# NVIDIA-Merlin/NVTabular

Hardware: AMD Instinct MI355X
Metric: rows/sec + GB/s (Criteo Categorify+FillMissing+Normalize fit+transform, HBM-resident) (higher is better)
Workload: dtype int32 keys -> int64 labels; fp64 moments/normalize; 1 GPU; synthetic Criteo-day0: 26 int32 categorical (Criteo-1TB cardinalities, Zipf) + 13 int32 continuous, nulls as Arrow bitmaps; Categorify + FillMissing + Normalize, fit + transform; rows_per_gpu=45000000, algorithmic_bytes_per_row=624, tie_break=value (count desc, value asc), artifacts=deferred (no parquet I/O inside the timed region)

## Files before the change

### nvtabular_amd/csrc/nvt_range_count.hip

```cpp
#include <cstdio>
#include <cstdlib>
#include <type_traits>

#include "nvt_common.hpp"
#include "nvt_internal.hpp"
#include "nvt_prof.hpp"
#include "nvt_range.hpp"

namespace nvt {

namespace {

constexpr int32_t kEmpty = INT32_MIN;
constexpr int kRpBS = 1024;
constexpr int kRpG = NVT_RANGE_WGS;
constexpr int kRpBinWords = 20480;
constexpr int kRpLine = 16;
constexpr int kRpMaxNbLog2 = 10;
constexpr int kHotSlotsR = NVT_HOT_IMAGE_WORDS;
constexpr int kHotBucketsR = kHotSlotsR / 2;
constexpr int kRpProbe = 512;
#ifndef NVT_RP_MAX_EPOCH
#define NVT_RP_MAX_EPOCH 8
#endif
constexpr unsigned kRpMaxEpoch = NVT_RP_MAX_EPOCH;
#ifndef NVT_RANGE_U
#define NVT_RANGE_U 2
#endif
constexpr unsigned long long kStAgg = 1ull << 62, kStPrefix = 2ull << 62,
                             kStMask = (1ull << 62) - 1ull;

__device__ __forceinline__ uint32_t hot_bucket_r(int32_t key) { return hot_image_bucket(key, kHotBucketsR - 1); }

template <bool PW>
__device__ __forceinline__ uint32_t rp_fine(const RangeMap &map, int32_t key) {
  if constexpr (PW) return map.fine(key);
  else return map.template fine_staged<false>(key);
}


template <int U, int NBL, bool PW>
__global__ __launch_bounds__(kRpBS) void rp_partition_kernel(
    const int32_t *__restrict__ keys, const uint8_t *__restrict__ valid, uint64_t n,
    const int32_t *__restrict__ aux, int nb_log2_rt, uint32_t region_cap, int32_t *__restrict__ regions,
    uint32_t *__restrict__ fills, unsigned *__restrict__ hot_cnt, uint64_t *state,
    unsigned long long *__restrict__ clr_status, unsigned *__restrict__ clr_hist) {
  const int nb_log2 = NBL ? NBL : nb_log2_rt;
  {
    const unsigned nst = (1u << nb_log2) + 8u;
    for (unsigned i = blockIdx.x * kRpBS + threadIdx.x; i < nst; i += kRpG * kRpBS) clr_status[i] = 0ull;
    if (blockIdx.x == kRpG - 1 && threadIdx.x < 256) clr_hist[threadIdx.x] = 0u;
  }
  __shared__ int4 hot[kHotBucketsR];
  __shared__ int32_t bins[kRpBinWords];
  __shared__ unsigned fill[1 << kRpMaxNbLog2], flushed[1 << kRpMaxNbLog2];
  __shared__ unsigned scratch[kWave];
  __shared__ unsigned long long s_nulls, s_sent;
  __shared__ unsigned s_ovf;
  const unsigned NB = 1u << nb_log2, CAP = (unsigned)kRpBinWords >> nb_log2;
  const unsigned g = blockIdx.x, lane = lane_id();
  int32_t fill0 = 0x5A5A5A5A, fill1 = fill0 + 1;
  while (hot_bucket_r(fill1) == hot_bucket_r(fill0)) ++fill1;
  const uint32_t fb0 = hot_bucket_r(fill0);
  for (int i = threadIdx.x; i < kHotBucketsR; i += kRpBS) {
    const int2 k2 = reinterpret_cast<const int2 *>(aux)[i];
    const int32_t fk = (uint32_t)i != fb0 ? fill0 : fill1;
    hot[i] = make_int4(k2.x == kEmpty ? fk : k2.x, k2.y == kEmpty ? fk : k2.y, 0, 0);
  }
  for (unsigned i = threadIdx.x; i < NB; i += kRpBS) {
    fill[i] = 0;
    flushed[i] = 0;
  }
  if (threadIdx.x == 0) {
    s_nulls = 0;
    s_sent = 0;
    s_ovf = 0;
  }
  RangeMap map = load_map(aux);
  __shared__ uint32_t s_pieces[kRpPwWords];
  stage_pieces(map, s_pieces, threadIdx.x, kRpBS);
  __syncthreads();

  const unsigned BPW = NB / (kRpBS / kWave);
  __shared__ unsigned s_epoch[2];
  if (threadIdx.x < 2) s_epoch[threadIdx.x] = 0;
  auto flush_bins = [&](bool all, unsigned parity) {
    {
      const bool owner = lane < BPW;
      const unsigned wave_base = (threadIdx.x / kWave) * BPW;
      const unsigned t = wave_base + (owner ? lane : 0u);
      const unsigned fr = owner ? fill[t] : 0u;
      const unsigned done0 = owner ? flushed[t] : 0u;
      const bool over = fr > CAP;
      const unsigned f = over ? CAP : fr;
      const unsigned nfl = (all || over) ? f : (f / kRpLine) * kRpLine;
      const unsigned padn = over ? ((0u - (done0 + fr)) & (kRpLine - 1u)) : 0u;
      {
        const unsigned long long ob = __ballot(over);
        const unsigned long long hb = __ballot(fr * 2u > CAP);
        if (lane == 0 && (ob | hb))
          atomicAdd(&s_epoch[parity], ((unsigned)__popcll(ob) << 8) | (hb ? 1u : 0u));
      }
      unsigned long long todo = __ballot(nfl > 0);
      const unsigned sub = lane >> 4, l16 = lane & 15;
      while (todo) {
        int sel = -1;
#pragma unroll
        for (unsigned q = 0; q < 4; ++q) {
          const int bit = todo ? (int)__ffsll((long long)todo) - 1 : -1;
          if (todo) todo &= todo - 1;
          sel = (q == sub) ? bit : sel;
        }
        const unsigned src = sel >= 0 ? (unsigned)sel : 0u;
        const unsigned fb = __shfl(f, src, 64), nb_out = __shfl(nfl, src, 64);
        const unsigned done = __shfl(done0, src, 64), frb = __shfl(fr, src, 64), pb = __shfl(padn, src, 64);
        if (sel >= 0) {
          const unsigned bin = wave_base + (unsigned)sel;
          const int32_t *bsrc = bins + bin * CAP;
          const unsigned reach = frb > fb ? done + frb + pb : done + nb_out;
          if (reach > region_cap) {
            if (l16 == 0) atomicOr(&s_ovf, 1u);
          } else {
            int32_t *dst = regions + ((uint64_t)bin * kRpG + g) * region_cap + done;
            for (unsigned u = l16; u < nb_out; u += kRpLine) dst[u] = bsrc[u];
            if (l16 < pb) dst[frb + l16] = kEmpty;
          }
          const unsigned rem = fb - nb_out;
          int32_t keep = 0;
          if (l16 < rem) keep = bsrc[nb_out + l16];
          if (l16 < rem) bins[bin * CAP + l16] = keep;
        }
      }
      if (owner) {
        fill[t] = f - nfl;
        flushed[t] = over ? done0 + fr + padn : done0 + nfl;
      }
    }
  };

  const uint64_t nvec = (n + 3) / 4, nfull = n / 4;
  const uint64_t per = (nvec + kRpG - 1) / kRpG;
  const uint64_t v_lo = (uint64_t)g * per;
  const uint64_t v_hi = v_lo + per < nvec ? v_lo + per : nvec;
  const uint64_t vf_hi = v_hi < nfull ? v_hi : nfull;
  unsigned long long nulls = 0, notvalid = 0;
  unsigned long long empties = 0;
  const uint8_t *vsrc = valid != nullptr ? valid : reinterpret_cast<const uint8_t *>(keys);
  const unsigned vor = valid != nullptr ? 0u : 0xFFu;
  const uint64_t v_last = vf_hi > v_lo ? vf_hi - 1 : 0;
  int4 npack[U];
  unsigned nbyte[U];
  auto issue = [&](uint64_t v0) {
#pragma unroll
    for (int u = 0; u < U; ++u) {
      uint64_t v = v0 + (uint64_t)u * kRpBS;
      v = v < v_last ? v : v_last;
      npack[u] = reinterpret_cast<const int4 *>(keys)[v];
      nbyte[u] = (unsigned)vsrc[v >> 1];
    }
  };
  bool tail_round = false;
  int4 tpack = make_int4(0, 0, 0, 0);
  unsigned tok = 0, tin = 0;
  if (nfull < nvec && nfull >= v_lo && nfull < v_hi) {
    tail_round = true;
    if (threadIdx.x == 0) {
      int32_t kk[4] = {0, 0, 0, 0};
      for (int j = 0; j < 4; ++j) {
        const uint64_t i = nfull * 4 + j;
        if (i < n) {
          tin |= 1u << j;
          if (bit_valid(valid, i)) {
            kk[j] = keys[i];
            tok |= 1u << j;
          }
        }
      }
      tpack = make_int4(kk[0], kk[1], kk[2], kk[3]);
    }
  }
  unsigned R = 1, since = 0, epoch = 0;
  if (vf_hi > v_lo) issue(v_lo + threadIdx.x);
  for (uint64_t v0 = v_lo; v0 < vf_hi || tail_round; v0 += (uint64_t)kRpBS * U) {
    const bool is_tail = !(v0 < vf_hi);
    int32_t kv[4 * U];
    unsigned oks[U], ins[U];
#pragma unroll
    for (int u = 0; u < U; ++u) {
      const uint64_t v = v0 + (uint64_t)u * kRpBS + threadIdx.x;
      const bool present = !is_tail && v < vf_hi;
      kv[4 * u + 0] = npack[u].x;
      kv[4 * u + 1] = npack[u].y;
      kv[4 * u + 2] = npack[u].z;
      kv[4 * u + 3] = npack[u].w;
      oks[u] = present ? (((nbyte[u] | vor) >> (((unsigned)v & 1u) * 4u)) & 0xFu) : 0u;
      ins[u] = present ? 0xFu : 0u;
    }
    if (is_tail) {
      tail_round = false;
      kv[0] = tpack.x;
      kv[1] = tpack.y;
      kv[2] = tpack.z;
      kv[3] = tpack.w;
      oks[0] = tok;
      ins[0] = tin;
    } else {
      issue(v0 + (uint64_t)kRpBS * U + threadIdx.x);
    }
    unsigned pend = 0;
#pragma unroll
    for (int u = 0; u < U; ++u) {
      const unsigned ok = oks[u], in = ins[u];
      nulls += __popc(in & ~ok);
      notvalid += 4u - __popc(ok);
      int32_t kp[4];
      int4 hb[4];
      uint32_t sa[4];
#pragma unroll
      for (int j = 0; j < 4; ++j) {
        const int32_t m = (int32_t)(ok << (31 - j)) >> 31;
        kp[j] = (kv[4 * u + j] & m) | (kEmpty & ~m);
        sa[j] = hot_bucket_r(kp[j]);
      }
#pragma unroll
      for (int j = 0; j < 4; ++j) {
        const int2 kk2 = *reinterpret_cast<const int2 *>(&hot[sa[j]]);
        hb[j].x = kk2.x;
        hb[j].y = kk2.y;
      }
#pragma unroll
      for (int j = 0; j < 4; ++j) {
        const int q = 4 * u + j;
        const int32_t key = kp[j];
        const bool hx = hb[j].x == key, hy = hb[j].y == key;
        const bool hit = hx | hy;
        const bool is_e = key == kEmpty;
        empties += (unsigned)__popcll(__ballot(is_e));
        unsigned *cnt = reinterpret_cast<unsigned *>(&hot[sa[j]]) + (hy ? 3 : 2);
        atomicAdd(hit ? cnt : &scratch[lane], hit ? 1u : 0u);
        pend |= ((!hit & !is_e) ? 1u : 0u) << q;
      }
    }
    if (s_ovf) pend = 0;
#pragma unroll
    for (int q = 0; q < 4 * U; ++q) {
      if ((pend >> q) & 1) {
        const unsigned bkt = rp_fine<PW>(map, kv[q]) >> 14;
        const unsigned pos = atomicAdd(&fill[bkt], 1u);
        if (pos < CAP) {
          bins[bkt * CAP + pos] = kv[q];
        } else {
          const unsigned at = flushed[bkt] + pos;
          if (at < region_cap)
            regions[((uint64_t)bkt * kRpG + g) * region_cap + at] = kv[q];
          else
            atomicOr(&s_ovf, 1u);
        }
      }
    }
    if (++since >= R) {
      __syncthreads();
      flush_bins(false, epoch & 1u);
      if (threadIdx.x == 0) s_epoch[(epoch + 1u) & 1u] = 0;
      __syncthreads();
      const unsigned fl = s_epoch[epoch & 1u];
#ifndef NVT_RP_GROW_DIV
#define NVT_RP_GROW_DIV 16u
#endif
#ifndef NVT_RP_SHRINK_DIV
#define NVT_RP_SHRINK_DIV 4u
#endif
      if ((fl >> 8) > NB / NVT_RP_SHRINK_DIV) R = R > 1u ? R / 2u : 1u;
      else if ((fl >> 8) <= NB / NVT_RP_GROW_DIV) R = R < kRpMaxEpoch ? R * 2u : R;
      ++epoch;
      since = 0;
    }
  }
  __syncthreads();
  flush_bins(true, epoch & 1u);
  __syncthreads();
  for (unsigned b = threadIdx.x; b < NB; b += kRpBS) fills[(uint64_t)b * kRpG + g] = flushed[b];
  for (int i = threadIdx.x; i < kHotBucketsR; i += kRpBS) {
    const int4 hbk = hot[i];
    reinterpret_cast<uint2 *>(hot_cnt + (uint64_t)g * kHotSlotsR)[i] = make_uint2((unsigned)hbk.z, (unsigned)hbk.w);
  }
#pragma unroll
  for (int off = 32; off > 0; off >>= 1) {
    nulls += __shfl_down(nulls, off, 64);
    notvalid += __shfl_down(notvalid, off, 64);
  }
  if (lane == 0) {
    if (nulls) atomicAdd(&s_nulls, nulls);
    const unsigned long long sent = empties - notvalid;
    if (sent) atomicAdd(&s_sent, sent);
  }
  __syncthreads();
  if (threadIdx.x == 0) {
    if (s_nulls) atomicAdd((unsigned long long *)&state[NVT_ST_NULLS], s_nulls);
    if (s_sent) atomicAdd((unsigned long long *)&state[NVT_ST_SENTINEL], s_sent);
    if (s_ovf) atomicOr((unsigned long long *)&state[NVT_ST_OVERFLOW], 1ull | NVT_OVF_REGION);
    if (g == 0) atomicAdd((unsigned long long *)&state[NVT_ST_ROWS], (unsigned long long)n);
  }
}

constexpr int kTotGroups = 16;
__global__ __launch_bounds__(64 * kTotGroups) void hot_totals_kernel(
    const unsigned *__restrict__ hot_cnt, int nblocks, unsigned *__restrict__ hot_tot) {
  __shared__ unsigned part[kTotGroups][64];
  const unsigned l = threadIdx.x & 63, g = threadIdx.x >> 6;
  const unsigned slot = blockIdx.x * 64 + l;
  unsigned t = 0;
#pragma unroll 16
  for (int b = (int)g; b < nblocks; b += kTotGroups) t += hot_cnt[(uint64_t)b * kHotSlotsR + slot];
  part[g][l] = t;
  __syncthreads();
  if (g != 0) return;
  unsigned tot = 0;
#pragma unroll
  for (int q = 0; q < kTotGroups; ++q) tot += part[q][l];
  hot_tot[slot] = tot;
}

template <bool PW>
__global__ __launch_bounds__(kRpBS) void rp_count_kernel(
    const int32_t *__restrict__ regions, const uint32_t *__restrict__ fills, uint32_t region_cap,
    const int32_t *__restrict__ aux, const unsigned *__restrict__ hot_tot, int nb_log2,
    unsigned long long *status, unsigned *ticket, int32_t *__restrict__ out_keys,
    int64_t *__restrict__ out_cnt, uint64_t out_cap, unsigned *cls_hist,
    unsigned long long *__restrict__ range_table, uint32_t *__restrict__ out_slots, uint64_t *state) {
  constexpr int NSL = kRpSlots + kRpTail;
  constexpr int NW = kRpBS / kWave;
  __shared__ int32_t lkeys[NSL];
  __shared__ unsigned lcnt[NSL];
  __shared__ unsigned run_len[kRpG];
  __shared__ unsigned hist[256];
  __shared__ unsigned wtot[NW];
  __shared__ unsigned lovf, s_b, s_bad, s_mx;
  __shared__ unsigned long long s_base;
  if (threadIdx.x == 0) {
    s_b = atomicAdd(ticket, 1u);
    lovf = 0;
    s_mx = 0;
  }
  for (int i = threadIdx.x; i < NSL; i += kRpBS) {
    lkeys[i] = kEmpty;
    lcnt[i] = 0;
  }
  if (threadIdx.x < 256) hist[threadIdx.x] = 0;
  __syncthreads();
  const unsigned b = s_b, NB = 1u << nb_log2;
  const unsigned lane = lane_id(), w = threadIdx.x / kWave;
  RangeMap map = load_map(aux);
  __shared__ uint32_t s_pieces[kRpPwWords];
  stage_pieces(map, s_pieces, threadIdx.x, kRpBS);
  const bool skip = (state[NVT_ST_OVERFLOW] & 1ull) != 0;
  if (threadIdx.x < kRpG) {
    const unsigned len = fills[(uint64_t)b * kRpG + threadIdx.x];
    run_len[threadIdx.x] = (skip || len > region_cap) ? 0u : len;
  }
  __syncthreads();
  bool failed = skip;
  auto insert_from = [&](int32_t key, unsigned wgt, uint32_t s) {
#pragma unroll 4
    for (int p = 0; p < kRpProbe; ++p, ++s) {
      if (s >= (uint32_t)NSL) break;
      int32_t cur = lkeys[s];
      if (cur == kEmpty) {
        cur = atomicCAS(&lkeys[s], kEmpty, key);
        if (cur == kEmpty) cur = key;
      }
      if (cur == key) {
        atomicAdd(&lcnt[s], wgt);
        return;
      }
    }
    failed = true;
  };
  const unsigned hot_h0 = (unsigned)aux[NVT_RANGE_AUX_HOTSTART + b], hot_h1 = (unsigned)aux[NVT_RANGE_AUX_HOTSTART + b + 1];
  int32_t hot_key0 = kEmpty;
  unsigned hot_tot0 = 0;
  if (hot_h0 + threadIdx.x < hot_h1) {
    const unsigned slot = reinterpret_cast<const unsigned short *>(aux + NVT_RANGE_AUX_HOTORDER)[hot_h0 + threadIdx.x];
    hot_key0 = aux[slot];
    hot_tot0 = hot_tot[slot];
  }
  {
    __shared__ unsigned s_pre[kRpG + 2];
    __shared__ unsigned s_wsum[kRpG / kWave];
    static_assert(kRpG % kWave == 0 && kRpG <= kRpBS, "one thread per run");
    {
      unsigned len = 0, inc = 0;
      if (threadIdx.x < kRpG) {
        len = run_len[threadIdx.x];
        inc = len;
#pragma unroll
        for (int off = 1; off < 64; off <<= 1) {
          const unsigned o = __shfl_up(inc, off, 64);
          if (lane >= (unsigned)off) inc += o;
        }
        if (lane == 63) s_wsum[w] = inc;
      }
      __syncthreads();
      if (threadIdx.x < kRpG) {
        unsigned wb = 0;
        for (unsigned q = 0; q < w; ++q) wb += s_wsum[q];
        s_pre[threadIdx.x] = wb + inc - len;
        if (threadIdx.x == kRpG - 1) s_pre[kRpG] = wb + inc;
      }
    }
    __syncthreads();
    const unsigned *pre = s_pre;
    const unsigned all_keys = pre[kRpG];
    const unsigned share = (all_keys + NW - 1) / NW;
    const unsigned f_lo = w * share < all_keys ? w * share : all_keys;
    const unsigned total = f_lo + share < all_keys ? f_lo + share : all_keys;
    const int32_t *rbase = regions + (uint64_t)b * kRpG * region_cap;
#ifndef NVT_RP_GB
#define NVT_RP_GB 8
#endif
    constexpr int GB = NVT_RP_GB;
    unsigned r = 0;
    {
      const unsigned f = f_lo + lane < all_keys ? f_lo + lane : (all_keys ? all_keys - 1 : 0);
      unsigned lo = 0, hi = kRpG;
      while (hi - lo > 1) {
        const unsigned mid = (lo + hi) >> 1;
        if (pre[mid] <= f) lo = mid; else hi = mid;
      }
      r = lo;
    }
    unsigned r_lo = pre[r], r_hi = pre[r + 1];
    for (unsigned f0 = f_lo; f0 < total && !failed; f0 += GB * kWave) {
      int32_t kk[GB];
#pragma unroll
      for (int u = 0; u < GB; ++u) {
        const unsigned f = f0 + u * kWave + lane;
        kk[u] = kEmpty;
        if (f < total) {
          while (f >= r_hi) {
            ++r;
            r_lo = r_hi;
            r_hi = pre[r + 1];
          }
          kk[u] = rbase[(uint64_t)r * region_cap + (f - r_lo)];
        }
      }
      uint32_t hs[GB];
      int32_t cur[GB];
#pragma unroll
      for (int u = 0; u < GB; ++u) hs[u] = rp_fine<PW>(map, kk[u]) & (kRpSlots - 1);
#pragma unroll
      for (int u = 0; u < GB; ++u) cur[u] = lkeys[hs[u]];
#pragma unroll
      for (int u = 0; u < GB; ++u) {
        if (cur[u] == kEmpty && kk[u] != kEmpty) {
          cur[u] = atomicCAS(&lkeys[hs[u]], kEmpty, kk[u]);
          cur[u] = cur[u] == kEmpty ? kk[u] : cur[u];
        }
      }
      unsigned todo = 0;
#pragma unroll
      for (int u = 0; u < GB; ++u) {
        if (kk[u] == kEmpty) continue;
        if (cur[u] == kk[u])
          atomicAdd(&lcnt[hs[u]], 1u);
        else
          todo |= 1u << u;
      }
      int32_t wkey = 0;
      uint32_t ws = 0;
      int wp = 0;
      bool walking = false;
      while (true) {
        if (!walking && todo) {
          const int u = (int)__ffs((int)todo) - 1;
          wkey = kk[0];
          ws = hs[0];
#pragma unroll
          for (int q = 1; q < GB; ++q) {
            wkey = u == q ? kk[q] : wkey;
            ws = u == q ? hs[q] : ws;
          }
          todo &= todo - 1u;
          ++ws;
          wp = 1;
          walking = true;
        }
        if (!__any(walking)) break;
        if (walking) {
          if (ws >= (uint32_t)NSL || wp >= kRpProbe) {
            failed = true;
            walking = false;
          } else {
            int32_t c = lkeys[ws];
            if (c == kEmpty) {
              c = atomicCAS(&lkeys[ws], kEmpty, wkey);
              if (c == kEmpty) c = wkey;
            }
            if (c == wkey) {
              atomicAdd(&lcnt[ws], 1u);
              walking = false;
            } else {
              ++ws;
              ++wp;
            }
          }
        }
      }
    }
  }
  {
    if (hot_key0 != kEmpty && hot_tot0 > 0 && !failed)
      insert_from(hot_key0, hot_tot0, rp_fine<PW>(map, hot_key0) & (kRpSlots - 1));
    const unsigned short *order = reinterpret_cast<const unsigned short *>(aux + NVT_RANGE_AUX_HOTORDER);
    for (unsigned jx = hot_h0 + threadIdx.x + kRpBS; jx < hot_h1; jx += kRpBS) {
      const unsigned slot = order[jx];
      const int32_t key = aux[slot];
      const unsigned tot = hot_tot[slot];
      if (key != kEmpty && tot > 0 && !failed) insert_from(key, tot, rp_fine<PW>(map, key) & (kRpSlots - 1));
    }
  }
  if (failed) atomicOr(&lovf, 1u);
  __syncthreads();
  if (threadIdx.x == 0)
    s_bad = (lovf != 0 ||
             (__hip_atomic_load(&state[NVT_ST_OVERFLOW], __ATOMIC_RELAXED,
                                __HIP_MEMORY_SCOPE_AGENT) & 1ull))
                ? 1u : 0u;
  __syncthreads();
  const bool bad = s_bad != 0;
  const unsigned long long sent_rows = b == 0 ? state[NVT_ST_SENTINEL] : 0ull;
  const unsigned extra = sent_rows > 0 ? 1u : 0u;
  constexpr int ITER = (NSL + kRpBS - 1) / kRpBS;
  unsigned mine = 0;
  for (int it = 0; it < ITER; ++it) {
    const int i = it * kRpBS + (int)threadIdx.x;
    const bool occ = i < NSL && lkeys[i] != kEmpty;
    mine += (unsigned)__popcll(__ballot(occ));
  }
  if (lane == 0) wtot[w] = mine;
  __syncthreads();
  unsigned E = extra;
  for (int q = 0; q < NW; ++q) E += wtot[q];
  const bool full = E > (unsigned)(kRpSlots / 4 * 3);
  if (bad || full) E = 0;
  if (w == 0) {
    unsigned long long excl = 0;
    if (lane == 0)
      __hip_atomic_store(&status[b], (b == 0 ? kStPrefix : kStAgg) | (unsigned long long)E,
                         __ATOMIC_RELAXED, __HIP_MEMORY_SCOPE_AGENT);
    if (b > 0) {
      int top = (int)b - 1;
      while (true) {
        const int idx = top - (int)lane;
        unsigned long long v = kStPrefix;
        if (idx >= 0) {
          do {
            v = __hip_atomic_load(&status[idx], __ATOMIC_RELAXED, __HIP_MEMORY_SCOPE_AGENT);
#ifndef NVT_RP_SLEEP
#define NVT_RP_SLEEP 1
#endif
            if ((v >> 62) == 0) __builtin_amdgcn_s_sleep(NVT_RP_SLEEP);
          } while ((v >> 62) == 0);
        }
        const unsigned long long isp = __ballot((v >> 62) == 2);
        const int first = isp ? (int)__ffsll((long long)isp) - 1 : 64;
        unsigned long long add = ((int)lane <= first) ? (v & kStMask) : 0ull;
#pragma unroll
        for (int off = 32; off > 0; off >>= 1) add += __shfl_down(add, off, 64);
        excl += __shfl(add, 0, 64);
        if (isp) break;
        top -= 64;
      }
      if (lane == 0)
        __hip_atomic_store(&status[b], kStPrefix | (excl + E), __ATOMIC_RELAXED,
                           __HIP_MEMORY_SCOPE_AGENT);
    }
    if (lane == 0) s_base = excl;
  }
  __syncthreads();
  const unsigned long long base = s_base;
  if (b == NB - 1 && threadIdx.x == 0) {
    if (base + E > out_cap) {
      atomicOr((unsigned long long *)&state[NVT_ST_OVERFLOW], 2ull);
      state[NVT_ST_NEED] = base + E;
    } else {
      state[NVT_ST_OCCUPIED] = base + E;
    }
  }
  if (bad || full) {
    if (threadIdx.x == 0 && (lovf != 0 || full))
      atomicOr((unsigned long long *)&state[NVT_ST_OVERFLOW],
               1ull | (lovf != 0 ? NVT_OVF_PROBE : 0ull) | (full ? NVT_OVF_FULL : 0ull));
    return;
  }
  if (base + E > out_cap) return;
  if (extra && threadIdx.x == 0) {
    out_keys[base] = kEmpty;
    out_cnt[base] = (int64_t)sent_rows;
    if (out_slots != nullptr) out_slots[base] = 0xFFFFFFFFu;
    const unsigned cls = sent_rows < 255 ? (unsigned)sent_rows : 255u;
    atomicAdd(&hist[cls], 1u);
    unsigned long long *gm = reinterpret_cast<unsigned long long *>(&state[NVT_ST_MAXCOUNT]);
    atomicMax(gm, sent_rows);
  }
  __shared__ unsigned occ_pre[ITER * NW];
  __shared__ unsigned occ_wsum[8];
  for (int it = 0; it < ITER; ++it) {
    const int i = it * kRpBS + (int)threadIdx.x;
    const bool occ = i < NSL && lkeys[i] != kEmpty;
    const unsigned c = (unsigned)__popcll(__ballot(occ));
    if (lane == 0) occ_pre[it * NW + w] = c;
  }
  __syncthreads();
  {
    constexpr int NG = ITER * NW;
    constexpr int SW = (NG + kWave - 1) / kWave;
    unsigned v = 0, inc = 0;
    if (w < (unsigned)SW) {
      v = threadIdx.x < (unsigned)NG ? occ_pre[threadIdx.x] : 0u;
      inc = v;
#pragma unroll
      for (int off = 1; off < 64; off <<= 1) {
        const unsigned o = __shfl_up(inc, off, 64);
        if (lane >= (unsigned)off) inc += o;
      }
      if (lane == 63) occ_wsum[w] = inc;
    }
    __syncthreads();
    if (w < (unsigned)SW && threadIdx.x < (unsigned)NG) {
      unsigned wb = 0;
      for (unsigned q = 0; q < w; ++q) wb += occ_wsum[q];
      occ_pre[threadIdx.x] = extra + wb + inc - v;
    }
    __syncthreads();
  }
  unsigned mx = 0;
  for (int it = 0; it < ITER; ++it) {
    const int i = it * kRpBS + (int)threadIdx.x;
    const int32_t k = i < NSL ? lkeys[i] : kEmpty;
    const bool occ = k != kEmpty;
    unsigned long long dump = kEncEmptySlot;
    const unsigned long long bal = __ballot(occ);
    const unsigned front = occ_pre[it * NW + w];
    if (occ) {
      const unsigned p_i = front + (unsigned)__popcll(bal & ((1ull << lane) - 1ull));
      unsigned rank = 0;
      int s = i;
      while (true) {
        int32_t o[4];
#pragma unroll
        for (int q = 0; q < 4; ++q) o[q] = s - 1 - q >= 0 ? lkeys[s - 1 - q] : kEmpty;
        int run = 0;
        bool open = true;
#pragma unroll
        for (int q = 0; q < 4; ++q) {
          open = open && o[q] != kEmpty;
          run += open ? 1 : 0;
          rank += (open && o[q] < k) ? 1u : 0u;
        }
        s -= run;
        if (run < 4) break;
      }
      int e = i + 1;
      while (true) {
        int32_t o[4];
#pragma unroll
        for (int q = 0; q < 4; ++q) o[q] = e + q < NSL ? lkeys[e + q] : kEmpty;
        int run = 0;
        bool open = true;
#pragma unroll
        for (int q = 0; q < 4; ++q) {
          open = open && o[q] != kEmpty;
          run += open ? 1 : 0;
          rank += (open && o[q] < k) ? 1u : 0u;
        }
        e += run;
        if (run < 4) break;
      }
      const uint64_t pos = base + p_i - (unsigned)(i - s) + rank;
      const unsigned c = lcnt[i];
      out_keys[pos] = k;
      out_cnt[pos] = (int64_t)c;
      if (out_slots != nullptr) out_slots[pos] = b * (unsigned)NSL + (unsigned)i;
      atomicAdd(&hist[c < 255u ? c : 255u], 1u);
      mx = c > mx ? c : mx;
      dump = ((unsigned long long)(uint32_t)pos << 32) | (uint32_t)k;
    }
    if (range_table != nullptr && i < NSL) range_table[(uint64_t)b * NSL + i] = dump;
  }
#pragma unroll
  for (int off = 32; off > 0; off >>= 1) {
    const unsigned o = __shfl_down(mx, off, 64);
    mx = o > mx ? o : mx;
  }
  if (lane == 0 && mx > 0) atomicMax(&s_mx, mx);
  if (range_table != nullptr && b == NB - 1 && threadIdx.x < kRpGuard)
    range_table[(uint64_t)NB * NSL + threadIdx.x] = kEncEmptySlot;
  __syncthreads();
  if (threadIdx.x == 0 && s_mx > 0)
    atomicMax(reinterpret_cast<unsigned long long *>(&state[NVT_ST_MAXCOUNT]), (unsigned long long)s_mx);
  if (threadIdx.x < 256) {
    const unsigned h = hist[threadIdx.x];
    if (h) atomicAdd(&cls_hist[threadIdx.x], h);
    if (threadIdx.x == 255 && h)
      atomicAdd((unsigned long long *)&state[NVT_ST_BIG], (unsigned long long)h);
  }
}

inline uint64_t al16(uint64_t x) { return (x + 15) & ~15ull; }

}

uint32_t range_region_cap(uint64_t n, int nb_log2) {
  const uint64_t rows_per_wg = (n + kRpG - 1) / kRpG;
  const uint64_t c = 2 * (rows_per_wg >> nb_log2) + 64;
  return (uint32_t)((c + kRpLine - 1) / kRpLine * kRpLine);
}

struct RangeWs {
  int32_t *regions;
  uint32_t *fills;
  unsigned *hot_cnt, *hot_tot;
  unsigned long long *status;
  unsigned *ticket;
};

uint64_t range_ws_layout(uint64_t n, int nb_log2, char *base, RangeWs *ws) {
  uint64_t off = 0;
  auto take = [&](uint64_t bytes) {
    char *p = base ? base + off : nullptr;
    off += al16(bytes);
    return p;
  };
  RangeWs w;
  const uint64_t NB = 1ull << nb_log2;
  w.regions = (int32_t *)take(NB * kRpG * range_region_cap(n, nb_log2) * 4);
  w.fills = (uint32_t *)take(NB * kRpG * 4);
  w.hot_cnt = (unsigned *)take((uint64_t)kRpG * kHotSlotsR * 4);
  w.hot_tot = (unsigned *)take((uint64_t)kHotSlotsR * 4);
  w.status = (unsigned long long *)take(NB * 8 + 64);
  w.ticket = (unsigned *)(w.status ? (char *)w.status + NB * 8 : nullptr);
  if (ws) *ws = w;
  return off;
}

uint64_t range_count_ws_bytes(uint64_t n, int nb_log2) {
  return range_ws_layout(n, nb_log2, nullptr, nullptr);
}

int range_count_i32(const int32_t *keys, const uint8_t *valid, uint64_t n, int nb_log2, void *wsp,
                    int32_t *aux, int32_t *out_keys, int64_t *out_cnt, uint64_t out_cap,
                    void *range_table, uint32_t *out_slots, uint64_t *state, hipStream_t s, bool pieces) {
  if (range_table == nullptr) out_slots = nullptr;
  NVT_CHECK_ARG(nb_log2 >= 6 && nb_log2 <= kRpMaxNbLog2, "range path: 64 .. 1024 buckets");
  NVT_CHECK_ARG(aux != nullptr, "range path: the column needs its aux block (hot_image)");
  NVT_PROF("dense_count_r9", n * 4, s);
  RangeWs w;
  range_ws_layout(n, nb_log2, (char *)wsp, &w);
  const unsigned NB = 1u << nb_log2;
  const uint32_t cap = range_region_cap(n, nb_log2);
  unsigned *hist = (unsigned *)(aux + NVT_RANGE_AUX_HIST);
#define NVT_RP_PART(NBL)                                                                            \
  do {                                                                                              \
    if (pieces)                                                                                     \
      rp_partition_kernel<NVT_RANGE_U, NBL, true><<<kRpG, kRpBS, 0, s>>>(                           \
          keys, valid, n, aux, nb_log2, cap, w.regions, w.fills, w.hot_cnt, state, w.status, hist); \
    else                                                                                            \
      rp_partition_kernel<NVT_RANGE_U, NBL, false><<<kRpG, kRpBS, 0, s>>>(                          \
          keys, valid, n, aux, nb_log2, cap, w.regions, w.fills, w.hot_cnt, state, w.status, hist); \
  } while (0)
  if (nb_log2 == 8) NVT_RP_PART(8);
  else if (nb_log2 == 9) NVT_RP_PART(9);
  else if (nb_log2 == 10) NVT_RP_PART(10);
  else NVT_RP_PART(0);
#undef NVT_RP_PART
  NVT_CHECK_LAUNCH();
  hot_totals_kernel<<<kHotSlotsR / 64, 64 * kTotGroups, 0, s>>>(w.hot_cnt, kRpG, w.hot_tot);
  NVT_CHECK_LAUNCH();
  if (pieces)
    rp_count_kernel<true><<<NB, kRpBS, 0, s>>>(w.regions, w.fills, cap, aux, w.hot_tot, nb_log2, w.status,
                                               w.ticket, out_keys, out_cnt, out_cap,
                                               (unsigned *)(aux + NVT_RANGE_AUX_HIST),
                                               (unsigned long long *)range_table, out_slots, state);
  else
    rp_count_kernel<false><<<NB, kRpBS, 0, s>>>(w.regions, w.fills, cap, aux, w.hot_tot, nb_log2, w.status,
                                                w.ticket, out_keys, out_cnt, out_cap,
                                                (unsigned *)(aux + NVT_RANGE_AUX_HIST),
                                                (unsigned long long *)range_table, out_slots, state);
  NVT_CHECK_LAUNCH();
  return NVT_OK;
}

}
```

Measured before the change: 5.062 billion rows/s.

## Make range count kernel persistent with ticketed buckets and prefetch of next bucket

Launches the range count kernel with one workgroup per CU instead of one per bucket. Each workgroup loops, taking bucket tickets and clearing its shared table between buckets. While the current bucket finishes, it prefetches the next bucket's run lengths, hot-key order and first key batch to hide global load latency. This cuts launch and workgroup startup cost and overlaps the decoupled-lookback scan with loads. In exchange, buckets within a workgroup are processed serially, the lookback chain could serialise more, and the kernel needs extra shared state and a cached CU-count query.

New measurement: 4.429 billion rows/s. 0.875x the previous value.

```diff
diff --git a/nvtabular_amd/csrc/nvt_range_count.hip b/nvtabular_amd/csrc/nvt_range_count.hip
--- a/nvtabular_amd/csrc/nvt_range_count.hip
+++ b/nvtabular_amd/csrc/nvt_range_count.hip
@@ -1,3 +1,4 @@
+#include <atomic>
 #include <cstdio>
 #include <cstdlib>
 #include <type_traits>
@@ -321,6 +322,9 @@
   hot_tot[slot] = tot;
 }
 
+#ifndef NVT_RP_GB
+#define NVT_RP_GB 8
+#endif
 template <bool PW>
 __global__ __launch_bounds__(kRpBS) void rp_count_kernel(
     const int32_t *__restrict__ regions, const uint32_t *__restrict__ fills, uint32_t region_cap,
@@ -330,374 +334,407 @@
     unsigned long long *__restrict__ range_table, uint32_t *__restrict__ out_slots, uint64_t *state) {
   constexpr int NSL = kRpSlots + kRpTail;
   constexpr int NW = kRpBS / kWave;
+  constexpr int GB = NVT_RP_GB;
+  constexpr int ITER = (NSL + kRpBS - 1) / kRpBS;
+  static_assert(kRpG % kWave == 0 && kRpG <= kRpBS && (kRpG & (kRpG - 1)) == 0, "one thread per run");
   __shared__ int32_t lkeys[NSL];
   __shared__ unsigned lcnt[NSL];
-  __shared__ unsigned run_len[kRpG];
+  __shared__ unsigned s_pre[kRpG + 2];
+  __shared__ unsigned s_wsum[kRpG / kWave];
   __shared__ unsigned hist[256];
   __shared__ unsigned wtot[NW];
+  __shared__ unsigned occ_pre[ITER * NW];
+  __shared__ unsigned occ_wsum[8];
   __shared__ unsigned lovf, s_b, s_bad, s_mx;
   __shared__ unsigned long long s_base;
+  __shared__ uint32_t s_pieces[kRpPwWords];
   if (threadIdx.x == 0) {
     s_b = atomicAdd(ticket, 1u);
     lovf = 0;
     s_mx = 0;
   }
-  for (int i = threadIdx.x; i < NSL; i += kRpBS) {
-    lkeys[i] = kEmpty;
-    lcnt[i] = 0;
-  }
+  auto clear_table = [&]() {
+    for (int i = threadIdx.x; i < NSL; i += kRpBS) {
+      lkeys[i] = kEmpty;
+      lcnt[i] = 0;
+    }
+  };
+  clear_table();
   if (threadIdx.x < 256) hist[threadIdx.x] = 0;
-  __syncthreads();
-  const unsigned b = s_b, NB = 1u << nb_log2;
+  const unsigned NB = 1u << nb_log2;
   const unsigned lane = lane_id(), w = threadIdx.x / kWave;
   RangeMap map = load_map(aux);
-  __shared__ uint32_t s_pieces[kRpPwWords];
   stage_pieces(map, s_pieces, threadIdx.x, kRpBS);
   const bool skip = (state[NVT_ST_OVERFLOW] & 1ull) != 0;
-  if (threadIdx.x < kRpG) {
-    const unsigned len = fills[(uint64_t)b * kRpG + threadIdx.x];
-    run_len[threadIdx.x] = (skip || len > region_cap) ? 0u : len;
-  }
-  __syncthreads();
-  bool failed = skip;
-  auto insert_from = [&](int32_t key, unsigned wgt, uint32_t s) {
-#pragma unroll 4
-    for (int p = 0; p < kRpProbe; ++p, ++s) {
-      if (s >= (uint32_t)NSL) break;
-      int32_t cur = lkeys[s];
-      if (cur == kEmpty) {
-        cur = atomicCAS(&lkeys[s], kEmpty, key);
-        if (cur == kEmpty) cur = key;
-      }
-      if (cur == key) {
-        atomicAdd(&lcnt[s], wgt);
-        return;
-      }
-    }
-    failed = true;
+  const unsigned short *order = reinterpret_cast<const unsigned short *>(aux + NVT_RANGE_AUX_HOTORDER);
+
+  unsigned n_len = 0, n_h0 = 0, n_h1 = 0, n_slot = 0, n_tot = 0;
+  int32_t n_key = kEmpty;
+  unsigned r = 0, r_lo = 0, r_hi = 0, f_lo = 0, total = 0;
+  const int32_t *rbase = regions;
+  int32_t kk[GB];
+  unsigned vm = 0;
+  auto load_batch = [&](unsigned f0) {
+    vm = 0;
+#pragma unroll
+    for (int u = 0; u < GB; ++u) {
+      const unsigned f = f0 + u * kWave + lane;
+      uint64_t at = 0;
+      if (f < total) {
+        while (f >= r_hi) {
+          ++r;
+          r_lo = r_hi;
+          r_hi = s_pre[r + 1];
+        }
+        at = (uint64_t)r * region_cap + (f - r_lo);
+        vm |= 1u << u;
+      }
+      kk[u] = rbase[at];
+    }
   };
-  const unsigned hot_h0 = (unsigned)aux[NVT_RANGE_AUX_HOTSTART + b], hot_h1 = (unsigned)aux[NVT_RANGE_AUX_HOTSTART + b + 1];
-  int32_t hot_key0 = kEmpty;
-  unsigned hot_tot0 = 0;
-  if (hot_h0 + threadIdx.x < hot_h1) {
-    const unsigned slot = reinterpret_cast<const unsigned short *>(aux + NVT_RANGE_AUX_HOTORDER)[hot_h0 + threadIdx.x];
-    hot_key0 = aux[slot];
-    hot_tot0 = hot_tot[slot];
-  }
-  {
-    __shared__ unsigned s_pre[kRpG + 2];
-    __shared__ unsigned s_wsum[kRpG / kWave];
-    static_assert(kRpG % kWave == 0 && kRpG <= kRpBS, "one thread per run");
-    {
-      unsigned len = 0, inc = 0;
-      if (threadIdx.x < kRpG) {
-        len = run_len[threadIdx.x];
-        inc = len;
-#pragma unroll
-        for (int off = 1; off < 64; off <<= 1) {
-          const unsigned o = __shfl_up(inc, off, 64);
-          if (lane >= (unsigned)off) inc += o;
-        }
-        if (lane == 63) s_wsum[w] = inc;
-      }
-      __syncthreads();
-      if (threadIdx.x < kRpG) {
-        unsigned wb = 0;
-        for (unsigned q = 0; q < w; ++q) wb += s_wsum[q];
-        s_pre[threadIdx.x] = wb + inc - len;
-        if (threadIdx.x == kRpG - 1) s_pre[kRpG] = wb + inc;
-      }
+  auto request_runs = [&](unsigned bx) {
+    unsigned bc = bx < NB ? bx : NB - 1u;
+    asm volatile("" : "+v"(bc));
+    n_len = fills[(uint64_t)bc * kRpG + (threadIdx.x & (kRpG - 1))];
+    n_h0 = (unsigned)aux[NVT_RANGE_AUX_HOTSTART + bc];
+    n_h1 = (unsigned)aux[NVT_RANGE_AUX_HOTSTART + bc + 1];
+  };
+  auto request_hot_order = [&]() {
+    const unsigned j = n_h0 + threadIdx.x;
+    n_slot = order[j < n_h1 ? j : 0u];
+  };
+  auto request_hot_keys = [&]() {
+    const unsigned slot = n_h0 + threadIdx.x < n_h1 ? n_slot : 0u;
+    n_key = aux[slot];
+    n_tot = hot_tot[slot];
+  };
+  auto request_first_batch = [&](unsigned bx) {
+    const unsigned bc = bx < NB ? bx : NB - 1u;
+    const unsigned len = (skip || bx >= NB || n_len > region_cap) ? 0u : n_len;
+    unsigned inc = len;
+    if (threadIdx.x < kRpG) {
+#pragma unroll
+      for (int off = 1; off < 64; off <<= 1) {
+        const unsigned o = __shfl_up(inc, off, 64);
+        if (lane >= (unsigned)off) inc += o;
+      }
+      if (lane == 63) s_wsum[w] = inc;
     }
     __syncthreads();
-    const unsigned *pre = s_pre;
-    const unsigned all_keys = pre[kRpG];
+    if (threadIdx.x < kRpG) {
+      unsigned wb = 0;
+      for (unsigned q = 0; q < w; ++q) wb += s_wsum[q];
+      s_pre[threadIdx.x] = wb + inc - len;
+      if (threadIdx.x == kRpG - 1) s_pre[kRpG] = wb + inc;
+    }
+    __syncthreads();
+    const unsigned all_keys = s_pre[kRpG];
     const unsigned share = (all_keys + NW - 1) / NW;
-    const unsigned f_lo = w * share < all_keys ? w * share : all_keys;
-    const unsigned total = f_lo + share < all_keys ? f_lo + share : all_keys;
-    const int32_t *rbase = regions + (uint64_t)b * kRpG * region_cap;
-#ifndef NVT_RP_GB
-#define NVT_RP_GB 8
-#endif
-    constexpr int GB = NVT_RP_GB;
-    unsigned r = 0;
+    f_lo = w * share < all_keys ? w * share : all_keys;
+    total = f_lo + share < all_keys ? f_lo + share : all_keys;
+    rbase = regions + (uint64_t)bc * kRpG * region_cap;
     {
       const unsigned f = f_lo + lane < all_keys ? f_lo + lane : (all_keys ? all_keys - 1 : 0);
       unsigned lo = 0, hi = kRpG;
       while (hi - lo > 1) {
         const unsigned mid = (lo + hi) >> 1;
-        if (pre[mid] <= f) lo = mid; else hi = mid;
+        if (s_pre[mid] <= f) lo = mid; else hi = mid;
       }
       r = lo;
     }
-    unsigned r_lo = pre[r], r_hi = pre[r + 1];
-    for (unsigned f0 = f_lo; f0 < total && !failed; f0 += GB * kWave) {
-      int32_t kk[GB];
-#pragma unroll
-      for (int u = 0; u < GB; ++u) {
-        const unsigned f = f0 + u * kWave + lane;
-        kk[u] = kEmpty;
-        if (f < total) {
-          while (f >= r_hi) {
-            ++r;
-            r_lo = r_hi;
-            r_hi = pre[r + 1];
+    r_lo = s_pre[r];
+    r_hi = s_pre[r + 1];
+    load_batch(f_lo);
+  };
+
+  __syncthreads();
+  unsigned b = s_b;
+  request_runs(b);
+  request_hot_order();
+  request_first_batch(b);
+  request_hot_keys();
+
+  while (b < NB) {
+    unsigned next_ticket = 0;
+    if (threadIdx.x == 0) next_ticket = atomicInc(ticket, 0xFFFFFFFFu);
+    bool failed = skip;
+    auto insert_from = [&](int32_t key, unsigned wgt, uint32_t s) {
+#pragma unroll 4
+      for (int p = 0; p < kRpProbe; ++p, ++s) {
+        if (s >= (uint32_t)NSL) break;
+        int32_t cur = lkeys[s];
+        if (cur == kEmpty) {
+          cur = atomicCAS(&lkeys[s], kEmpty, key);
+          if (cur == kEmpty) cur = key;
+        }
+        if (cur == key) {
+          atomicAdd(&lcnt[s], wgt);
+          return;
+        }
+      }
+      failed = true;
+    };
+    {
+      for (unsigned f0 = f_lo; f0 < total && !failed; f0 += GB * kWave) {
+        if (f0 != f_lo) load_batch(f0);
+#pragma unroll
+        for (int u = 0; u < GB; ++u) kk[u] = ((vm >> u) & 1u) ? kk[u] : kEmpty;
+        uint32_t hs[GB];
+        int32_t cur[GB];
+#pragma unroll
+        for (int u = 0; u < GB; ++u) hs[u] = rp_fine<PW>(map, kk[u]) & (kRpSlots - 1);
+#pragma unroll
+        for (int u = 0; u < GB; ++u) cur[u] = lkeys[hs[u]];
+#pragma unroll
+        for (int u = 0; u < GB; ++u) {
+          if (cur[u] == kEmpty && kk[u] != kEmpty) {
+            cur[u] = atomicCAS(&lkeys[hs[u]], kEmpty, kk[u]);
+            cur[u] = cur[u] == kEmpty ? kk[u] : cur[u];
           }
-          kk[u] = rbase[(uint64_t)r * region_cap + (f - r_lo)];
-        }
-      }
-      uint32_t hs[GB];
-      int32_t cur[GB];
-#pragma unroll
-      for (int u = 0; u < GB; ++u) hs[u] = rp_fine<PW>(map, kk[u]) & (kRpSlots - 1);
-#pragma unroll
-      for (int u = 0; u < GB; ++u) cur[u] = lkeys[hs[u]];
-#pragma unroll
-      for (int u = 0; u < GB; ++u) {
-        if (cur[u] == kEmpty && kk[u] != kEmpty) {
-          cur[u] = atomicCAS(&lkeys[hs[u]], kEmpty, kk[u]);
-          cur[u] = cur[u] == kEmpty ? kk[u] : cur[u];
-        }
-      }
-      unsigned todo = 0;
-#pragma unroll
-      for (int u = 0; u < GB; ++u) {
-        if (kk[u] == kEmpty) continue;
-        if (cur[u] == kk[u])
-          atomicAdd(&lcnt[hs[u]], 1u);
-        else
-          todo |= 1u << u;
-      }
-      int32_t wkey = 0;
-      uint32_t ws = 0;
-      int wp = 0;
-      bool walking = false;
-      while (true) {
-        if (!walking && todo) {
-          const int u = (int)__ffs((int)todo) - 1;
-          wkey = kk[0];
-          ws = hs[0];
-#pragma unroll
-          for (int q = 1; q < GB; ++q) {
-            wkey = u == q ? kk[q] : wkey;
-            ws = u == q ? hs[q] : ws;
+        }
+        unsigned todo = 0;
+#pragma unroll
+        for (int u = 0; u < GB; ++u) {
+          if (kk[u] == kEmpty) continue;
+          if (cur[u] == kk[u])
+            atomicAdd(&lcnt[hs[u]], 1u);
+          else
+            todo |= 1u << u;
+        }
+        int32_t wkey = 0;
+        uint32_t ws = 0;
+        int wp = 0;
+        bool walking = false;
+        while (true) {
+          if (!walking && todo) {
+            const int u = (int)__ffs((int)todo) - 1;
+            wkey = kk[0];
+            ws = hs[0];
+#pragma unroll
+            for (int q = 1; q < GB; ++q) {
+              wkey = u == q ? kk[q] : wkey;
+              ws = u == q ? hs[q] : ws;
+            }
+            todo &= todo - 1u;
+            ++ws;
+            wp = 1;
+            walking = true;
           }
-          todo &= todo - 1u;
-          ++ws;
-          wp = 1;
-          walking = true;
-        }
-        if (!__any(walking)) break;
-        if (walking) {
-          if (ws >= (uint32_t)NSL || wp >= kRpProbe) {
-            failed = true;
-            walking = false;
-          } else {
-            int32_t c = lkeys[ws];
-            if (c == kEmpty) {
-              c = atomicCAS(&lkeys[ws], kEmpty, wkey);
-              if (c == kEmpty) c = wkey;
-            }
-            if (c == wkey) {
-              atomicAdd(&lcnt[ws], 1u);
+          if (!__any(walking)) break;
+          if (walking) {
+            if (ws >= (uint32_t)NSL || wp >= kRpProbe) {
+              failed = true;
               walking = false;
             } else {
-              ++ws;
-              ++wp;
+              int32_t c = lkeys[ws];
+              if (c == kEmpty) {
+                c = atomicCAS(&lkeys[ws], kEmpty, wkey);
+                if (c == kEmpty) c = wkey;
+              }
+              if (c == wkey) {
+                atomicAdd(&lcnt[ws], 1u);
+                walking = false;
+              } else {
+                ++ws;
+                ++wp;
+              }
             }
           }
         }
       }
     }
-  }
-  {
-    if (hot_key0 != kEmpty && hot_tot0 > 0 && !failed)
-      insert_from(hot_key0, hot_tot0, rp_fine<PW>(map, hot_key0) & (kRpSlots - 1));
-    const unsigned short *order = reinterpret_cast<const unsigned short *>(aux + NVT_RANGE_AUX_HOTORDER);
-    for (unsigned jx = hot_h0 + threadIdx.x + kRpBS; jx < hot_h1; jx += kRpBS) {
-      const unsigned slot = order[jx];
-      const int32_t key = aux[slot];
-      const unsigned tot = hot_tot[slot];
-      if (key != kEmpty && tot > 0 && !failed) insert_from(key, tot, rp_fine<PW>(map, key) & (kRpSlots - 1));
-    }
-  }
-  if (failed) atomicOr(&lovf, 1u);
-  __syncthreads();
-  if (threadIdx.x == 0)
-    s_bad = (lovf != 0 ||
-             (__hip_atomic_load(&state[NVT_ST_OVERFLOW], __ATOMIC_RELAXED,
-                                __HIP_MEMORY_SCOPE_AGENT) & 1ull))
-                ? 1u : 0u;
-  __syncthreads();
-  const bool bad = s_bad != 0;
-  const unsigned long long sent_rows = b == 0 ? state[NVT_ST_SENTINEL] : 0ull;
-  const unsigned extra = sent_rows > 0 ? 1u : 0u;
-  constexpr int ITER = (NSL + kRpBS - 1) / kRpBS;
-  unsigned mine = 0;
-  for (int it = 0; it < ITER; ++it) {
-    const int i = it * kRpBS + (int)threadIdx.x;
-    const bool occ = i < NSL && lkeys[i] != kEmpty;
-    mine += (unsigned)__popcll(__ballot(occ));
-  }
-  if (lane == 0) wtot[w] = mine;
-  __syncthreads();
-  unsigned E = extra;
-  for (int q = 0; q < NW; ++q) E += wtot[q];
-  const bool full = E > (unsigned)(kRpSlots / 4 * 3);
-  if (bad || full) E = 0;
-  if (w == 0) {
-    unsigned long long excl = 0;
-    if (lane == 0)
-      __hip_atomic_store(&status[b], (b == 0 ? kStPrefix : kStAgg) | (unsigned long long)E,
-                         __ATOMIC_RELAXED, __HIP_MEMORY_SCOPE_AGENT);
-    if (b > 0) {
-      int top = (int)b - 1;
-      while (true) {
-        const int idx = top - (int)lane;
-        unsigned long long v = kStPrefix;
-        if (idx >= 0) {
-          do {
-            v = __hip_atomic_load(&status[idx], __ATOMIC_RELAXED, __HIP_MEMORY_SCOPE_AGENT);
+    {
+      if (n_h0 + threadIdx.x < n_h1 && n_key != kEmpty && n_tot > 0 && !failed)
+        insert_from(n_key, n_tot, rp_fine<PW>(map, n_key) & (kRpSlots - 1));
+      for (unsigned jx = n_h0 + threadIdx.x + kRpBS; jx < n_h1; jx += kRpBS) {
+        const unsigned slot = order[jx];
+        const int32_t key = aux[slot];
+        const unsigned tot = hot_tot[slot];
+        if (key != kEmpty && tot > 0 && !failed) insert_from(key, tot, rp_fine<PW>(map, key) & (kRpSlots - 1));
+      }
+    }
+    if (failed) atomicOr(&lovf, 1u);
+    if (threadIdx.x == 0) s_b = next_ticket;
+    __syncthreads();
+    const unsigned bn = s_b;
+    request_runs(bn);
+    unsigned ovf_bits = 0;
+    if (threadIdx.x == 0)
+      ovf_bits = __hip_atomic_load(reinterpret_cast<const unsigned *>(&state[NVT_ST_OVERFLOW]), __ATOMIC_RELAXED,
+                                   __HIP_MEMORY_SCOPE_AGENT);
+    const unsigned long long sent_rows = b == 0 ? state[NVT_ST_SENTINEL] : 0ull;
+    const unsigned extra = sent_rows > 0 ? 1u : 0u;
+    unsigned mine = 0;
+    for (int it = 0; it < ITER; ++it) {
+      const int i = it * kRpBS + (int)threadIdx.x;
+      const bool occ = i < NSL && lkeys[i] != kEmpty;
+      const unsigned c = (unsigned)__popcll(__ballot(occ));
+      if (lane == 0) occ_pre[it * NW + w] = c;
+      mine += c;
+    }
+    if (lane == 0) wtot[w] = mine;
+    asm volatile("" : "+v"(ovf_bits));
+    if (threadIdx.x == 0) s_bad = (lovf != 0 || (ovf_bits & 1u)) ? 1u : 0u;
+    __syncthreads();
+    const bool bad = s_bad != 0;
+    request_hot_order();
+    unsigned E = extra;
+    for (int q = 0; q < NW; ++q) E += wtot[q];
+    const bool full = E > (unsigned)(kRpSlots / 4 * 3);
+    if (bad || full) E = 0;
+    if (w == 0) {
+      unsigned long long excl = 0;
+      if (lane == 0)
+        __hip_atomic_store(&status[b], (b == 0 ? kStPrefix : kStAgg) | (unsigned long long)E,
+                           __ATOMIC_RELAXED, __HIP_MEMORY_SCOPE_AGENT);
+      if (b > 0) {
+        int top = (int)b - 1;
+        while (true) {
+          const int idx = top - (int)lane;
+          unsigned long long v = kStPrefix;
+          if (idx >= 0) {
+            do {
+              v = __hip_atomic_load(&status[idx], __ATOMIC_RELAXED, __HIP_MEMORY_SCOPE_AGENT);
 #ifndef NVT_RP_SLEEP
 #define NVT_RP_SLEEP 1
 #endif
-            if ((v >> 62) == 0) __builtin_amdgcn_s_sleep(NVT_RP_SLEEP);
-          } while ((v >> 62) == 0);
-        }
-        const unsigned long long isp = __ballot((v >> 62) == 2);
-        const int first = isp ? (int)__ffsll((long long)isp) - 1 : 64;
-        unsigned long long add = ((int)lane <= first) ? (v & kStMask) : 0ull;
-#pragma unroll
-        for (int off = 32; off > 0; off >>= 1) add += __shfl_down(add, off, 64);
-        excl += __shfl(add, 0, 64);
-        if (isp) break;
-        top -= 64;
-      }
-      if (lane == 0)
-        __hip_atomic_store(&status[b], kStPrefix | (excl + E), __ATOMIC_RELAXED,
-                           __HIP_MEMORY_SCOPE_AGENT);
-    }
-    if (lane == 0) s_base = excl;
-  }
-  __syncthreads();
-  const unsigned long long base = s_base;
-  if (b == NB - 1 && threadIdx.x == 0) {
-    if (base + E > out_cap) {
-      atomicOr((unsigned long long *)&state[NVT_ST_OVERFLOW], 2ull);
-      state[NVT_ST_NEED] = base + E;
-    } else {
-      state[NVT_ST_OCCUPIED] = base + E;
-    }
-  }
-  if (bad || full) {
-    if (threadIdx.x == 0 && (lovf != 0 || full))
-      atomicOr((unsigned long long *)&state[NVT_ST_OVERFLOW],
-               1ull | (lovf != 0 ? NVT_OVF_PROBE : 0ull) | (full ? NVT_OVF_FULL : 0ull));
-    return;
-  }
-  if (base + E > out_cap) return;
-  if (extra && threadIdx.x == 0) {
-    out_keys[base] = kEmpty;
-    out_cnt[base] = (int64_t)sent_rows;
-    if (out_slots != nullptr) out_slots[base] = 0xFFFFFFFFu;
-    const unsigned cls = sent_rows < 255 ? (unsigned)sent_rows : 255u;
-    atomicAdd(&hist[cls], 1u);
-    unsigned long long *gm = reinterpret_cast<unsigned long long *>(&state[NVT_ST_MAXCOUNT]);
-    atomicMax(gm, sent_rows);
-  }
-  __shared__ unsigned occ_pre[ITER * NW];
-  __shared__ unsigned occ_wsum[8];
-  for (int it = 0; it < ITER; ++it) {
-    const int i = it * kRpBS + (int)threadIdx.x;
-    const bool occ = i < NSL && lkeys[i] != kEmpty;
-    const unsigned c = (unsigned)__popcll(__ballot(occ));
-    if (lane == 0) occ_pre[it * NW + w] = c;
-  }
-  __syncthreads();
-  {
-    constexpr int NG = ITER * NW;
-    constexpr int SW = (NG + kWave - 1) / kWave;
-    unsigned v = 0, inc = 0;
-    if (w < (unsigned)SW) {
-      v = threadIdx.x < (unsigned)NG ? occ_pre[threadIdx.x] : 0u;
-      inc = v;
-#pragma unroll
-      for (int off = 1; off < 64; off <<= 1) {
-        const unsigned o = __shfl_up(inc, off, 64);
-        if (lane >= (unsigned)off) inc += o;
-      }
-      if (lane == 63) occ_wsum[w] = inc;
+              if ((v >> 62) == 0) __builtin_amdgcn_s_sleep(NVT_RP_SLEEP);
+            } while ((v >> 62) == 0);
+          }
+          const unsigned long long isp = __ballot((v >> 62) == 2);
+          const int first = isp ? (int)__ffsll((long long)isp) - 1 : 64;
+          unsigned long long add = ((int)lane <= first) ? (v & kStMask) : 0ull;
+#pragma unroll
+          for (int off = 32; off > 0; off >>= 1) add += __shfl_down(add, off, 64);
+          excl += __shfl(add, 0, 64);
+          if (isp) break;
+          top -= 64;
+        }
+        if (lane == 0)
+          __hip_atomic_store(&status[b], kStPrefix | (excl + E), __ATOMIC_RELAXED,
+                             __HIP_MEMORY_SCOPE_AGENT);
+      }
+      if (lane == 0) s_base = excl;
     }
     __syncthreads();
-    if (w < (unsigned)SW && threadIdx.x < (unsigned)NG) {
-      unsigned wb = 0;
-      for (unsigned q = 0; q < w; ++q) wb += occ_wsum[q];
-      occ_pre[threadIdx.x] = extra + wb + inc - v;
+    const unsigned long long base = s_base;
+    if (b == NB - 1 && threadIdx.x == 0) {
+      if (base + E > out_cap) {
+        atomicOr((unsigned long long *)&state[NVT_ST_OVERFLOW], 2ull);
+        state[NVT_ST_NEED] = base + E;
+      } else {
+        state[NVT_ST_OCCUPIED] = base + E;
+      }
+    }
+    if (bad || full) {
+      if (threadIdx.x == 0 && (lovf != 0 || full))
+        atomicOr((unsigned long long *)&state[NVT_ST_OVERFLOW],
+                 1ull | (lovf != 0 ? NVT_OVF_PROBE : 0ull) | (full ? NVT_OVF_FULL : 0ull));
+    }
+    const bool emit = !(bad || full) && base + E <= out_cap;
+    request_first_batch(bn);
+    request_hot_keys();
+    if (emit) {
+      if (extra && threadIdx.x == 0) {
+        out_keys[base] = kEmpty;
+        out_cnt[base] = (int64_t)sent_rows;
+        if (out_slots != nullptr) out_slots[base] = 0xFFFFFFFFu;
+        const unsigned cls = sent_rows < 255 ? (unsigned)sent_rows : 255u;
+        atomicAdd(&hist[cls], 1u);
+        unsigned long long *gm = reinterpret_cast<unsigned long long *>(&state[NVT_ST_MAXCOUNT]);
+        atomicMax(gm, sent_rows);
+      }
+      {
+        constexpr int NG = ITER * NW;
+        constexpr int SW = (NG + kWave - 1) / kWave;
+        unsigned v = 0, inc = 0;
+        if (w < (unsigned)SW) {
+          v = threadIdx.x < (unsigned)NG ? occ_pre[threadIdx.x] : 0u;
+          inc = v;
+#pragma unroll
+          for (int off = 1; off < 64; off <<= 1) {
+            const unsigned o = __shfl_up(inc, off, 64);
+            if (lane >= (unsigned)off) inc += o;
+          }
+          if (lane == 63) occ_wsum[w] = inc;
+        }
+        __syncthreads();
+        if (w < (unsigned)SW && threadIdx.x < (unsigned)NG) {
+          unsigned wb = 0;
+          for (unsigned q = 0; q < w; ++q) wb += occ_wsum[q];
+          occ_pre[threadIdx.x] = extra + wb + inc - v;
+        }
+        __syncthreads();
+      }
+      unsigned mx = 0;
+      for (int it = 0; it < ITER; ++it) {
+        const int i = it * kRpBS + (int)threadIdx.x;
+        const int32_t k = i < NSL ? lkeys[i] : kEmpty;
+        const bool occ = k != kEmpty;
+        unsigned long long dump = kEncEmptySlot;
+        const unsigned long long bal = __ballot(occ);
+        const unsigned front = occ_pre[it * NW + w];
+        if (occ) {
+          const unsigned p_i = front + (unsigned)__popcll(bal & ((1ull << lane) - 1ull));
+          unsigned rank = 0;
+          int s = i;
+          while (true) {
+            int32_t o[4];
+#pragma unroll
+            for (int q = 0; q < 4; ++q) o[q] = s - 1 - q >= 0 ? lkeys[s - 1 - q] : kEmpty;
+            int run = 0;
+            bool open = true;
+#pragma unroll
+            for (int q = 0; q < 4; ++q) {
+              open = open && o[q] != kEmpty;
+              run += open ? 1 : 0;
+              rank += (open && o[q] < k) ? 1u : 0u;
+            }
+            s -= run;
+            if (run < 4) break;
+          }
+          int e = i + 1;
+          while (true) {
+            int32_t o[4];
+#pragma unroll
+            for (int q = 0; q < 4; ++q) o[q] = e + q < NSL ? lkeys[e + q] : kEmpty;
+            int run = 0;
+            bool open = true;
+#pragma unroll
+            for (int q = 0; q < 4; ++q) {
+              open = open && o[q] != kEmpty;
+              run += open ? 1 : 0;
+              rank += (open && o[q] < k) ? 1u : 0u;
+            }
+            e += run;
+            if (run < 4) break;
+          }
+          const uint64_t pos = base + p_i - (unsigned)(i - s) + rank;
+          const unsigned c = lcnt[i];
+          out_keys[pos] = k;
+          out_cnt[pos] = (int64_t)c;
+          if (out_slots != nullptr) out_slots[pos] = b * (unsigned)NSL + (unsigned)i;
+          atomicAdd(&hist[c < 255u ? c : 255u], 1u);
+          mx = c > mx ? c : mx;
+          dump = ((unsigned long long)(uint32_t)pos << 32) | (uint32_t)k;
+        }
+        if (range_table != nullptr && i < NSL) range_table[(uint64_t)b * NSL + i] = dump;
+      }
+#pragma unroll
+      for (int off = 32; off > 0; off >>= 1) {
+        const unsigned o = __shfl_down(mx, off, 64);
+        mx = o > mx ? o : mx;
+      }
+      if (lane == 0 && mx > 0) atomicMax(&s_mx, mx);
+      if (range_table != nullptr && b == NB - 1 && threadIdx.x < kRpGuard)
+        range_table[(uint64_t)NB * NSL + threadIdx.x] = kEncEmptySlot;
     }
     __syncthreads();
-  }
-  unsigned mx = 0;
-  for (int it = 0; it < ITER; ++it) {
-    const int i = it * kRpBS + (int)threadIdx.x;
-    const int32_t k = i < NSL ? lkeys[i] : kEmpty;
-    const bool occ = k != kEmpty;
-    unsigned long long dump = kEncEmptySlot;
-    const unsigned long long bal = __ballot(occ);
-    const unsigned front = occ_pre[it * NW + w];
-    if (occ) {
-      const unsigned p_i = front + (unsigned)__popcll(bal & ((1ull << lane) - 1ull));
-      unsigned rank = 0;
-      int s = i;
-      while (true) {
-        int32_t o[4];
-#pragma unroll
-        for (int q = 0; q < 4; ++q) o[q] = s - 1 - q >= 0 ? lkeys[s - 1 - q] : kEmpty;
-        int run = 0;
-        bool open = true;
-#pragma unroll
-        for (int q = 0; q < 4; ++q) {
-          open = open && o[q] != kEmpty;
-          run += open ? 1 : 0;
-          rank += (open && o[q] < k) ? 1u : 0u;
-        }
-        s -= run;
-        if (run < 4) break;
-      }
-      int e = i + 1;
-      while (true) {
-        int32_t o[4];
-#pragma unroll
-        for (int q = 0; q < 4; ++q) o[q] = e + q < NSL ? lkeys[e + q] : kEmpty;
-        int run = 0;
-        bool open = true;
-#pragma unroll
-        for (int q = 0; q < 4; ++q) {
-          open = open && o[q] != kEmpty;
-          run += open ? 1 : 0;
-          rank += (open && o[q] < k) ? 1u : 0u;
-        }
-        e += run;
-        if (run < 4) break;
-      }
-      const uint64_t pos = base + p_i - (unsigned)(i - s) + rank;
-      const unsigned c = lcnt[i];
-      out_keys[pos] = k;
-      out_cnt[pos] = (int64_t)c;
-      if (out_slots != nullptr) out_slots[pos] = b * (unsigned)NSL + (unsigned)i;
-      atomicAdd(&hist[c < 255u ? c : 255u], 1u);
-      mx = c > mx ? c : mx;
-      dump = ((unsigned long long)(uint32_t)pos << 32) | (uint32_t)k;
-    }
-    if (range_table != nullptr && i < NSL) range_table[(uint64_t)b * NSL + i] = dump;
-  }
-#pragma unroll
-  for (int off = 32; off > 0; off >>= 1) {
-    const unsigned o = __shfl_down(mx, off, 64);
-    mx = o > mx ? o : mx;
-  }
-  if (lane == 0 && mx > 0) atomicMax(&s_mx, mx);
-  if (range_table != nullptr && b == NB - 1 && threadIdx.x < kRpGuard)
-    range_table[(uint64_t)NB * NSL + threadIdx.x] = kEncEmptySlot;
-  __syncthreads();
+    if (bn < NB) clear_table();
+    if (threadIdx.x == 0) lovf = 0;
+    __syncthreads();
+    b = bn;
+  }
   if (threadIdx.x == 0 && s_mx > 0)
     atomicMax(reinterpret_cast<unsigned long long *>(&state[NVT_ST_MAXCOUNT]), (unsigned long long)s_mx);
   if (threadIdx.x < 256) {
@@ -747,6 +784,24 @@
 
 uint64_t range_count_ws_bytes(uint64_t n, int nb_log2) {
   return range_ws_layout(n, nb_log2, nullptr, nullptr);
+}
+
+static hipError_t range_count_cus(unsigned *cus) {
+  constexpr int kMaxDev = 64;
+  static std::atomic<unsigned> known[kMaxDev];
+  int dev = 0;
+  hipError_t e = hipGetDevice(&dev);
+  if (e != hipSuccess) return e;
+  unsigned n = dev < kMaxDev ? known[dev].load(std::memory_order_relaxed) : 0u;
+  if (n == 0) {
+    int v = 0;
+    e = hipDeviceGetAttribute(&v, hipDeviceAttributeMultiprocessorCount, dev);
+    if (e != hipSuccess) return e;
+    n = v > 0 ? (unsigned)v : 1u;
+    if (dev < kMaxDev) known[dev].store(n, std::memory_order_relaxed);
+  }
+  *cus = n;
+  return hipSuccess;
 }
 
 int range_count_i32(const int32_t *keys, const uint8_t *valid, uint64_t n, int nb_log2, void *wsp,
@@ -778,16 +833,19 @@
   NVT_CHECK_LAUNCH();
   hot_totals_kernel<<<kHotSlotsR / 64, 64 * kTotGroups, 0, s>>>(w.hot_cnt, kRpG, w.hot_tot);
   NVT_CHECK_LAUNCH();
+  unsigned cus = 0;
+  NVT_CHECK_HIP(range_count_cus(&cus));
+  const unsigned grid = NB < cus ? NB : cus;
   if (pieces)
-    rp_count_kernel<true><<<NB, kRpBS, 0, s>>>(w.regions, w.fills, cap, aux, w.hot_tot, nb_log2, w.status,
-                                               w.ticket, out_keys, out_cnt, out_cap,
-                                               (unsigned *)(aux + NVT_RANGE_AUX_HIST),
-                                               (unsigned long long *)range_table, out_slots, state);
+    rp_count_kernel<true><<<grid, kRpBS, 0, s>>>(w.regions, w.fills, cap, aux, w.hot_tot, nb_log2, w.status,
+                                                 w.ticket, out_keys, out_cnt, out_cap,
+                                                 (unsigned *)(aux + NVT_RANGE_AUX_HIST),
+                                                 (unsigned long long *)range_table, out_slots, state);
   else
-    rp_count_kernel<false><<<NB, kRpBS, 0, s>>>(w.regions, w.fills, cap, aux, w.hot_tot, nb_log2, w.status,
-                                                w.ticket, out_keys, out_cnt, out_cap,
-                                                (unsigned *)(aux + NVT_RANGE_AUX_HIST),
-                                                (unsigned long long *)range_table, out_slots, state);
+    rp_count_kernel<false><<<grid, kRpBS, 0, s>>>(w.regions, w.fills, cap, aux, w.hot_tot, nb_log2, w.status,
+                                                  w.ticket, out_keys, out_cnt, out_cap,
+                                                  (unsigned *)(aux + NVT_RANGE_AUX_HIST),
+                                                  (unsigned long long *)range_table, out_slots, state);
   NVT_CHECK_LAUNCH();
   return NVT_OK;
 }
```
